# ariloytynoja/pagan2-msa

Measured on AMD Instinct MI355X. Metric: DP cells/sec, 32x100 kb DNA progressive align (hot path in dependency order: fill + traceback per tree level), higher is better.
Workload: dtype f64; 1 GPU; cfg4_32x100kb_dna_anchored; leaves=32, length=100000, data_type=dna, anchors=prefix, offset 15, node_alignments=31, order=guide-tree levels one after the other (a parent needs its children)

## Files before the change

### include/pagan_dp.h

```cpp
#ifndef PAGAN_DP_H
#define PAGAN_DP_H

#include <stdint.h>

#ifdef __cplusplus
extern "C" {
#endif

#define PAGAN_OK              0
#define PAGAN_E_ARG          -1
#define PAGAN_E_GRAPH        -2
#define PAGAN_E_BAND         -3
#define PAGAN_E_MODEL        -4
#define PAGAN_E_NODEVICE     -5
#define PAGAN_E_NOMEM        -6
#define PAGAN_E_INTERNAL     -7
#define PAGAN_DP_REACHED      0
#define PAGAN_DP_UNREACHABLE  1

#define PAGAN_OPT_NO_TERMINAL_EDGES        1u
#define PAGAN_OPT_NO_REDUCED_TERMINAL_PEN  2u

enum { PAGAN_X_MAT = 0, PAGAN_Y_MAT = 1, PAGAN_M_MAT = 2 };
enum { PAGAN_MATCHED = 2, PAGAN_XGAPPED = 3, PAGAN_YGAPPED = 4,
// ... 80 lines not shown

typedef struct pagan_batch pagan_batch;

int  pagan_batch_create(int32_t n, const pagan_job *jobs, const pagan_opts *opts,
                        pagan_batch **out);
int  pagan_batch_run(pagan_batch *b);
int  pagan_batch_sync(pagan_batch *b);
int  pagan_batch_fetch(pagan_batch *b, pagan_result *out );
int  pagan_batch_last_ms(pagan_batch *b, double ms[2]);
int  pagan_batch_last_ms_detail(pagan_batch *b, double ms[6]);
int64_t pagan_batch_cells(const pagan_batch *b);
void pagan_batch_destroy(pagan_batch *b);
int  pagan_batch_debug_trace(pagan_batch *b, int32_t k, void *dst, int64_t bytes);
int  pagan_dp_debug_plan(const pagan_graph *left, const pagan_graph *right, const pagan_band *band,
                         uint8_t *cls, int32_t n_cls, int32_t *sched, int32_t sched_cap, int32_t *sched_len,
                         int32_t *lead_req );
int  pagan_dp_debug_far(const pagan_graph *left, const pagan_graph *right, const pagan_band *band,
                        uint8_t *hfL, uint8_t *hfR, uint8_t *hbit, uint8_t *cls);
int  pagan_dp_debug_strips(const pagan_graph *left, const pagan_graph *right, const pagan_band *band, int32_t max_sites,
                           int32_t *strips , int32_t cap, int64_t *desc_off ,
                           int64_t *desc , int64_t desc_cap);
int  pagan_dp_debug_tiles(const pagan_graph *left, const pagan_graph *right, const pagan_band *band,
                          int32_t *tiles , int32_t cap, int32_t *tile_side);
int  pagan_dp_debug_tiles_staircase(const int32_t *tiles, int32_t n);
int  pagan_dp_debug_compact(const pagan_graph *left, const pagan_graph *right, const pagan_band *band, int32_t *keep_left,
                            int32_t *keep_right, int32_t *slot_left, int32_t *slot_right, int32_t *upper, int32_t *lower,
                            int32_t *n_out);
int  pagan_dp_debug_route(const pagan_graph *left, const pagan_graph *right, const pagan_model *model, const pagan_band *band,
                          int32_t *n_out);
int  pagan_batch_debug_scores(pagan_batch *b, int32_t k, double *dst, int64_t count);
int  pagan_batch_debug_backptrs(pagan_batch *b, int32_t k, uint32_t *dst, int64_t count);
int  pagan_batch_debug_poison(pagan_batch *b);
int  pagan_batch_debug_followed(pagan_batch *b, int32_t k, int32_t *counts);
int  pagan_batch_debug_poke_bp(pagan_batch *b, int32_t k, int32_t i, int32_t j, int32_t vit, uint32_t word);
int  pagan_batch_debug_reruns(pagan_batch *b);

void    pagan_dp_release_cache(void);
int64_t pagan_dp_cached_device_bytes(int32_t device);

typedef struct pagan_model_prob {
    int32_t      n_states;
    const float *score;
    float        gap_open;
    float        gap_ext;
    float        non_gap;
} pagan_model_prob;

typedef struct pagan_fb pagan_fb;

int  pagan_fb_run(const pagan_graph *left, const pagan_graph *right, const pagan_model_prob *model,
                  const pagan_band *band, const pagan_opts *opts, pagan_fb **out);
int  pagan_fb_run_batch(int32_t n, const pagan_graph *const *left, const pagan_graph *const *right,
                        const pagan_model_prob *const *model, const pagan_band *const *band, const pagan_opts *opts,
                        pagan_fb **out);
int  pagan_fb_totals(const pagan_fb *fb, double *log_fwd, double *log_bwd, int64_t *cells);
int  pagan_fb_kernel_ms(const pagan_fb *fb, double ms[2]);
int  pagan_fb_groups(const pagan_fb *fb);
int  pagan_fb_schedule(const pagan_fb *fb);
int  pagan_fb_debug_route(const pagan_graph *left, const pagan_graph *right, const pagan_band *band, int32_t info[8]);
int  pagan_fb_dump(pagan_fb *fb, int32_t which, double *dst);
int  pagan_fb_posterior_cells(pagan_fb *fb, int32_t n, const int32_t *cells, double *post);
int  pagan_fb_sample_path(pagan_fb *fb, const double *u, int32_t n_u, pagan_result *out,
                          int32_t *visited, int32_t *n_visited);
void pagan_fb_destroy(pagan_fb *fb);

const char *pagan_dp_version(void);
// ... 6 lines not shown
```

### pagan2-msa_amd/__init__.py

```python
import ctypes as C
import os

from . import abi
from .abi import Band, Graph, Model, ModelProb, Result

_HERE = os.path.dirname(os.path.abspath(__file__))
LIB_PATH = os.environ.get("PAGAN_DP_LIB") or os.path.join(_HERE, "libpagan_dp.so")
_lib = None


class PaganError(RuntimeError):
    def __init__(self, code, what):
        super().__init__("%s failed with code %d" % (what, code))
        self.code = code


def lib():
    global _lib
    if _lib is None:
        if not os.path.exists(LIB_PATH):
            raise RuntimeError("libpagan_dp.so is missing: run `python -c 'import __graft_entry__ as g; g.build()'`")
        _lib = abi.declare(C.CDLL(LIB_PATH))
    return _lib

# ... 268 lines not shown
        ms = (C.c_double * 2)()
        _check(self._L.pagan_batch_last_ms(self._h, ms), "pagan_batch_last_ms")
        return ms[0], ms[1]

    def fetch(self):
        res = (abi.CResult * self.n)()
        rc = self._L.pagan_batch_fetch(self._h, res)
        try:
            _check(rc, "pagan_batch_fetch")
            return [Result(r) for r in res]
        finally:
            for r in res:
                self._L.pagan_result_free(C.byref(r))

    def debug_scores(self, k):
        import numpy as np
        out = np.empty((self.cells_of(k), 3), np.float64)
        _check(self._L.pagan_batch_debug_scores(self._h, k, out.ctypes.data_as(C.POINTER(C.c_double)), out.size),
               "pagan_batch_debug_scores")
        return out

    def debug_backptrs(self, k):
        import numpy as np
        out = np.empty((self.cells_of(k), 3), np.uint32)
        _check(self._L.pagan_batch_debug_backptrs(self._h, k, out.ctypes.data_as(C.POINTER(C.c_uint32)), out.size),
               "pagan_batch_debug_backptrs")
        return out

    def debug_followed(self, k):
        c = (C.c_int32 * 2)()
        _check(self._L.pagan_batch_debug_followed(self._h, k, c), "pagan_batch_debug_followed")
        return int(c[0]), int(c[1])

    def debug_poke_bp(self, k, i, j, vit, word):
        _check(self._L.pagan_batch_debug_poke_bp(self._h, k, i, j, vit, word), "pagan_batch_debug_poke_bp")

    def debug_reruns(self):
        return int(self._L.pagan_batch_debug_reruns(self._h))

    def debug_trace(self, k, n_cells):
        import numpy as np
        out = np.empty((n_cells, 3), np.int32)
        _check(self._L.pagan_batch_debug_trace(self._h, k, out.ctypes.data_as(C.c_void_p), out.nbytes), "pagan_batch_debug_trace")
        return out

    def cells_of(self, k):
        left, right, _, band = self.jobs[k]
        return self._L.pagan_dp_count_cells(left.n_sites, right.n_sites, C.byref(band.c) if band is not None else None)

    def close(self):
        if self._h:
            self._L.pagan_batch_destroy(self._h)
            self._h = C.c_void_p()

    def __del__(self):
        try:
            self.close()
        except Exception:
            pass
```

### pagan2-msa_amd/abi.py

```python
import ctypes as C

import numpy as np

PAGAN_OK = 0
PAGAN_E_ARG, PAGAN_E_GRAPH, PAGAN_E_BAND, PAGAN_E_MODEL = -1, -2, -3, -4
PAGAN_E_NODEVICE, PAGAN_E_NOMEM, PAGAN_E_INTERNAL = -5, -6, -7
PAGAN_DP_REACHED, PAGAN_DP_UNREACHABLE = 0, 1
OPT_NO_TERMINAL_EDGES = 1
OPT_NO_REDUCED_TERMINAL_PEN = 2
X_MAT, Y_MAT, M_MAT = 0, 1, 2
MATCHED, XGAPPED, YGAPPED, XSKIPPED, YSKIPPED = 2, 3, 4, 5, 6

_i32p = C.POINTER(C.c_int32)
_f32p = C.POINTER(C.c_float)


class CGraph(C.Structure):
    _fields_ = [("n_sites", C.c_int32), ("n_edges", C.c_int32), ("state", _i32p), ("bwd_off", _i32p),
                ("bwd_src", _i32p), ("bwd_logw", _f32p), ("bwd_eid", _i32p)]


class CModel(C.Structure):
    _fields_ = [("n_states", C.c_int32), ("log_score", _f32p), ("log_gap_open", C.c_float),
                ("log_gap_ext", C.c_float), ("log_gap_end_ext", C.c_float), ("log_non_gap", C.c_float)]
# ... 145 lines not shown
    lib.pagan_batch_sync.restype = C.c_int
    lib.pagan_batch_fetch.argtypes = [C.c_void_p, rp]
    lib.pagan_batch_fetch.restype = C.c_int
    lib.pagan_batch_last_ms.argtypes = [C.c_void_p, C.POINTER(C.c_double)]
    lib.pagan_batch_last_ms.restype = C.c_int
    lib.pagan_batch_last_ms_detail.argtypes = [C.c_void_p, C.POINTER(C.c_double)]
    lib.pagan_batch_last_ms_detail.restype = C.c_int
    lib.pagan_batch_cells.argtypes = [C.c_void_p]
    lib.pagan_batch_cells.restype = C.c_int64
    lib.pagan_batch_destroy.argtypes = [C.c_void_p]
    lib.pagan_batch_destroy.restype = None
    lib.pagan_batch_debug_trace.argtypes = [C.c_void_p, C.c_int32, C.c_void_p, C.c_int64]
    lib.pagan_batch_debug_trace.restype = C.c_int
    lib.pagan_dp_debug_plan.argtypes = [gp, gp, bp, C.POINTER(C.c_uint8), C.c_int32, _i32p, C.c_int32, _i32p, _i32p]
    lib.pagan_dp_debug_plan.restype = C.c_int
    lib.pagan_dp_debug_far.argtypes = [gp, gp, bp] + [C.POINTER(C.c_uint8)] * 4
    lib.pagan_dp_debug_far.restype = C.c_int
    lib.pagan_dp_debug_strips.argtypes = [gp, gp, bp, C.c_int32, _i32p, C.c_int32, C.POINTER(C.c_int64), C.POINTER(C.c_int64), C.c_int64]
    lib.pagan_dp_debug_strips.restype = C.c_int
    lib.pagan_dp_debug_tiles.argtypes = [gp, gp, bp, _i32p, C.c_int32, _i32p]
    lib.pagan_dp_debug_tiles.restype = C.c_int
    lib.pagan_dp_debug_compact.argtypes = [gp, gp, bp, _i32p, _i32p, _i32p, _i32p, _i32p, _i32p, _i32p]
    lib.pagan_dp_debug_compact.restype = C.c_int
    lib.pagan_dp_debug_tiles_staircase.argtypes = [_i32p, C.c_int32]
    lib.pagan_dp_debug_tiles_staircase.restype = C.c_int
    lib.pagan_dp_debug_route.argtypes = [gp, gp, C.POINTER(CModel), bp, _i32p]
    lib.pagan_dp_debug_route.restype = C.c_int
    lib.pagan_batch_debug_scores.argtypes = [C.c_void_p, C.c_int32, C.POINTER(C.c_double), C.c_int64]
    lib.pagan_batch_debug_scores.restype = C.c_int
    lib.pagan_batch_debug_backptrs.argtypes = [C.c_void_p, C.c_int32, C.POINTER(C.c_uint32), C.c_int64]
    lib.pagan_batch_debug_backptrs.restype = C.c_int
    lib.pagan_batch_debug_followed.argtypes = [C.c_void_p, C.c_int32, C.POINTER(C.c_int32)]
    lib.pagan_batch_debug_followed.restype = C.c_int
    lib.pagan_batch_debug_poke_bp.argtypes = [C.c_void_p, C.c_int32, C.c_int32, C.c_int32, C.c_int32, C.c_uint32]
    lib.pagan_batch_debug_poke_bp.restype = C.c_int
    lib.pagan_batch_debug_reruns.argtypes = [C.c_void_p]
    lib.pagan_batch_debug_reruns.restype = C.c_int
    lib.pagan_batch_debug_poison.argtypes = [C.c_void_p]
    lib.pagan_batch_debug_poison.restype = C.c_int
    lib.pagan_dp_release_cache.argtypes = []
    lib.pagan_dp_release_cache.restype = None
    lib.pagan_dp_cached_device_bytes.argtypes = [C.c_int32]
    lib.pagan_dp_cached_device_bytes.restype = C.c_int64
    mpp, f64p = C.POINTER(CModelProb), C.POINTER(C.c_double)
    lib.pagan_fb_run.argtypes = [gp, gp, mpp, bp, op, C.POINTER(C.c_void_p)]
    lib.pagan_fb_run.restype = C.c_int
    lib.pagan_fb_run_batch.argtypes = [C.c_int32, C.POINTER(gp), C.POINTER(gp), C.POINTER(mpp), C.POINTER(bp), op, C.POINTER(C.c_void_p)]
    lib.pagan_fb_run_batch.restype = C.c_int
    lib.pagan_fb_totals.argtypes = [C.c_void_p, f64p, f64p, C.POINTER(C.c_int64)]
    lib.pagan_fb_totals.restype = C.c_int
    lib.pagan_fb_kernel_ms.argtypes = [C.c_void_p, C.POINTER(C.c_double)]
    lib.pagan_fb_kernel_ms.restype = C.c_int
    lib.pagan_fb_groups.argtypes = [C.c_void_p]
    lib.pagan_fb_groups.restype = C.c_int
    lib.pagan_fb_schedule.argtypes = [C.c_void_p]
    lib.pagan_fb_schedule.restype = C.c_int
    lib.pagan_fb_debug_route.argtypes = [gp, gp, bp, _i32p]
    lib.pagan_fb_debug_route.restype = C.c_int
    lib.pagan_fb_dump.argtypes = [C.c_void_p, C.c_int32, f64p]
    lib.pagan_fb_dump.restype = C.c_int
    lib.pagan_fb_posterior_cells.argtypes = [C.c_void_p, C.c_int32, _i32p, f64p]
    lib.pagan_fb_posterior_cells.restype = C.c_int
    lib.pagan_fb_sample_path.argtypes = [C.c_void_p, f64p, C.c_int32, rp, _i32p, _i32p]
    lib.pagan_fb_sample_path.restype = C.c_int
    lib.pagan_fb_destroy.argtypes = [C.c_void_p]
    lib.pagan_fb_destroy.restype = None
    lib.pagan_dp_version.argtypes = []
    lib.pagan_dp_version.restype = C.c_char_p
    return lib


EXPORTED = ["pagan_dp_align", "pagan_dp_align_batch", "pagan_result_free", "pagan_dp_predict_bytes",
            "pagan_dp_count_cells", "pagan_dp_device_count", "pagan_dp_select_device", "pagan_batch_create",
            "pagan_batch_run", "pagan_batch_sync", "pagan_batch_fetch", "pagan_batch_last_ms",
            "pagan_batch_cells", "pagan_batch_last_ms_detail", "pagan_batch_destroy", "pagan_batch_debug_trace", "pagan_dp_debug_plan", "pagan_dp_debug_far", "pagan_dp_debug_strips", "pagan_dp_debug_tiles", "pagan_dp_debug_compact", "pagan_dp_debug_tiles_staircase", "pagan_dp_release_cache", "pagan_dp_cached_device_bytes", "pagan_dp_debug_route", "pagan_batch_debug_scores", "pagan_batch_debug_backptrs", "pagan_batch_debug_poison", "pagan_batch_debug_followed", "pagan_batch_debug_poke_bp", "pagan_batch_debug_reruns",
            "pagan_fb_run", "pagan_fb_run_batch", "pagan_fb_totals", "pagan_fb_kernel_ms", "pagan_fb_groups", "pagan_fb_schedule", "pagan_fb_debug_route", "pagan_fb_dump", "pagan_fb_posterior_cells", "pagan_fb_sample_path",
            "pagan_fb_destroy", "pagan_dp_version"]
```

### pagan2-msa_amd/csrc/dp_abi.hip

```cpp
#include <hip/hip_runtime.h>

#include <algorithm>
#include <atomic>
#include <thread>
#include <chrono>
#include <cmath>
#include <cstdint>
#include <cstdio>
#include <cstdlib>
#include <cstring>
#include <condition_variable>
#include <mutex>
#include <new>
#include <type_traits>
#include <vector>
#include <unordered_map>

#include "host_anchors.h"
#include "host_graph.h"
#include "../../include/pagan_dp.h"
#include "dp_device.h"
#include "dp_band.h"

template <int BLOCK> __global__ void pg_fill_wavefront(const PgDevJob *jobs, const int *which, unsigned flags);
// ... 1007 lines not shown
        if (!p) return;
        std::lock_guard<std::mutex> g(m);
        idle.emplace_back(p, cap);
    }
};
StagePool stage_pool;
struct Stage {
    char *p = nullptr;
    size_t cap = 0;
    explicit Stage(size_t n) { p = stage_pool.take(n, &cap); }
    ~Stage() { stage_pool.give(p, cap); }
    Stage(const Stage &) = delete;
    Stage &operator=(const Stage &) = delete;
    char *data() { return p; }
};

template <class T> void put(Stage &stage, const void *devptr_as_off, const T *src, size_t count) {
    if (count) std::memcpy(stage.data() + reinterpret_cast<size_t>(devptr_as_off), src, sizeof(T) * count);
}

static int bp_diags_per_block(int max_nd, int other_dims) {
    int dpb = PG_BP_DIAGS;
    while (dpb > 4 && (long long)((max_nd + dpb - 1) / dpb) * other_dims < 4096) dpb /= 2;
    return dpb;
}

int launch_fill(pagan_batch *b) {
    unsigned chk_banded = PG_FLAG_SCORE_CHECK, chk_wide = b->n_striped > 0 ? PG_FLAG_SCORE_CHECK : 0u;
    if (const char *e = std::getenv("PAGAN_DP_SCORE_CHECK")) {
        if (std::strcmp(e, "0") == 0) { chk_banded = 0; chk_wide = 0; }
        else if (std::strcmp(e, "all") == 0) chk_wide = PG_FLAG_SCORE_CHECK;
    }
    const unsigned spread = b->strips_spread ? PG_FLAG_STRIPS_SPREAD : 0u;
    hipStream_t tile_stream = nullptr;
    static std::atomic<int> n_cu_dev[64];
    bool ev3_recorded = false;
    if (b->n_striped > 0 && b->strips_alone) {
        HIP_TRY(hipMemsetAsync(b->arena.dev + b->sfollow_begin, 0, b->sfollow_bytes, b->stream));
        if (b->strip_grid > 0)
            hipLaunchKernelGGL((pg_fill_pipe<true, true>), dim3(b->strip_grid), dim3(pg_pipe_block()), 0, b->stream,
                               b->d_jobs, b->d_swhich, ((b->flags & 0x400u) ? b->flags : (b->flags & ~0x800u)) | spread, b->strip_grid);
        if (b->strip_grid_big > 0)
            hipLaunchKernelGGL((pg_fill_pipe<false, true>), dim3(b->strip_grid_big), dim3(pg_pipe_block()), 0, b->stream,
                               b->d_jobs, b->d_swhich + b->strip_grid, ((b->flags & 0x400u) ? b->flags : (b->flags & ~0x800u)) | spread, b->strip_grid_big);
    }
    if (b->n_striped > 0 && b->tile_off.size() <= 1) {
        hipStream_t st = b->stream;
        if (b->stream2) {
            HIP_TRY(hipEventRecord(b->ev_fork, b->stream));
            HIP_TRY(hipStreamWaitEvent(b->stream2, b->ev_fork, 0));
            st = b->stream2;
        }
        tile_stream = st;
    }
    if (b->tile_off.size() > 1) {
        static std::atomic<bool> tiles_set_dev[64];
        std::atomic<bool> &tiles_set = tiles_set_dev[b->device & 63];
        if (!tiles_set.load()) {
            HIP_TRY(hipFuncSetAttribute(reinterpret_cast<const void *>(pg_fill_tiles),
                                        hipFuncAttributeMaxDynamicSharedMemorySize, (int)pg_tiles_lds_bytes()));
            HIP_TRY(hipFuncSetAttribute(reinterpret_cast<const void *>(pg_fill_tiles_flow),
                                        hipFuncAttributeMaxDynamicSharedMemorySize, (int)pg_tiles_lds_bytes()));
            int n_cu = 0;
            HIP_TRY(hipDeviceGetAttribute(&n_cu, hipDeviceAttributeMultiprocessorCount, b->device));
            n_cu_dev[b->device & 63].store(n_cu > 0 ? n_cu : 256);
            tiles_set.store(true);
        }
        hipStream_t st = b->stream;
        if (b->stream2) {
            HIP_TRY(hipEventRecord(b->ev_fork, b->stream));
            HIP_TRY(hipStreamWaitEvent(b->stream2, b->ev_fork, 0));
            st = b->stream2;
        }
        tile_stream = st;
    }
    if (b->n_ring > 0) {
        static std::atomic<bool> lds_set_dev[64];
        std::atomic<bool> &lds_set = lds_set_dev[b->device & 63];
        if (!lds_set.load()) {
            HIP_TRY(hipFuncSetAttribute(reinterpret_cast<const void *>(pg_fill_ring<true>),
                                        hipFuncAttributeMaxDynamicSharedMemorySize, (int)pg_ring_lds_bytes()));
            HIP_TRY(hipFuncSetAttribute(reinterpret_cast<const void *>(pg_fill_ring<false>),
                                        hipFuncAttributeMaxDynamicSharedMemorySize, (int)pg_ring_lds_bytes()));
            lds_set.store(true);
        }
        const int n_small = b->n_ring_small, n_big = b->n_ring - b->n_ring_small;
        HIP_TRY(hipEventRecord(b->evk[0], b->stream)); b->evk_set[0] = true;
        if (b->use_pipe) {
            bool follow = b->bp_pass == 1 && b->follow_bytes > 0 && !b->no_follow;
            if (const char *f = std::getenv("PAGAN_DP_FOLLOW")) follow = follow && std::strcmp(f, "0") != 0;
            if (b->follow_bytes > 0) HIP_TRY(hipMemsetAsync(b->arena.dev + b->follow_begin, 0, b->follow_bytes, b->stream));
            auto followers = [&](int n_fill) { return follow && n_fill <= 32 ? std::min(96, 48 * ((n_fill + 7) / 8)) : 0; };
            if (n_small > 0)
                hipLaunchKernelGGL((pg_fill_pipe<true, false>), dim3(n_small + followers(n_small)), dim3(pg_pipe_block()), 0 , b->stream,
                                   b->d_jobs, b->d_which, b->flags | chk_banded, n_small);
            if (n_big > 0)
                hipLaunchKernelGGL((pg_fill_pipe<false, false>), dim3(n_big + followers(n_big)), dim3(pg_pipe_block()), 0, b->stream,
                                   b->d_jobs, b->d_which + n_small, b->flags | chk_banded, n_big);
            HIP_TRY(hipEventRecord(b->evk[1], b->stream)); b->evk_set[1] = true;
            if (b->bp_pass) {
                int max_nd = 1, max_w = 1;
                for (int k = 0; k < b->n; ++k) if (b->jobs[k].ring_ok) { max_nd = std::max(max_nd, b->dj[k].nd); max_w = std::max(max_w, b->jobs[k].dx.max_width); }
                const int zc = (max_w + PG_BP_CELLS - 1) / PG_BP_CELLS, dpb = bp_diags_per_block(max_nd, b->n_ring * zc);
                hipLaunchKernelGGL(pg_backptr, dim3((max_nd + dpb - 1) / dpb, b->n_ring, zc), dim3(256), 0, b->stream,
                                   b->d_jobs, b->d_which, (b->flags & 0xffu) | (b->bp_pass == 2 ? 0x100u : chk_banded), dpb);
                HIP_TRY(hipEventRecord(b->evk[2], b->stream)); b->evk_set[2] = true;
            }
        } else {
            b->evk_set[1] = false;
            if (n_small > 0)
                hipLaunchKernelGGL(pg_fill_ring<true>, dim3(n_small), dim3(576), pg_ring_lds_bytes(), b->stream,
                                   b->d_jobs, b->d_which, b->flags);
            if (n_big > 0)
                hipLaunchKernelGGL(pg_fill_ring<false>, dim3(n_big), dim3(576), pg_ring_lds_bytes(), b->stream,
                                   b->d_jobs, b->d_which + n_small, b->flags);
        }
    }
    if (b->n_wide > 0) {
        dim3 grid(b->n_wide);
        const int *which = b->d_which + b->n_ring;
        switch (b->block) {
        case 64: hipLaunchKernelGGL(pg_fill_wavefront<64>, grid, dim3(64), 0, b->stream, b->d_jobs, which, b->flags); break;
        case 256: hipLaunchKernelGGL(pg_fill_wavefront<256>, grid, dim3(256), 0, b->stream, b->d_jobs, which, b->flags); break;
        default: hipLaunchKernelGGL(pg_fill_wavefront<1024>, grid, dim3(1024), 0, b->stream, b->d_jobs, which, b->flags); break;
        }
        HIP_TRY(hipEventRecord(b->evk[5], b->stream)); b->evk_set[5] = true;
    }
    if (b->n_striped > 0 && !b->strips_alone) {
        HIP_TRY(hipEventRecord(b->evk[3], tile_stream)); b->evk_set[3] = true; ev3_recorded = true;
        HIP_TRY(hipMemsetAsync(b->arena.dev + b->sfollow_begin, 0, b->sfollow_bytes, tile_stream));
        if (b->strip_grid > 0)
// ... 934 lines not shown
    });
    int first_err = PAGAN_OK;
    for (int k = 0; k < b->n; ++k)
        if (rcs[k] != PAGAN_OK && first_err == PAGAN_OK) first_err = rcs[k];
    return first_err;
}

int pagan_batch_debug_poison(pagan_batch *b) {
    if (!b) return PAGAN_E_ARG;
    HIP_TRY(hipMemsetAsync(b->arena.dev + b->out_begin, 0xFF, b->arena.size - b->out_begin, b->stream));
    return PAGAN_OK;
}

int pagan_batch_debug_poke_bp(pagan_batch *b, int32_t k, int32_t i, int32_t j, int32_t vit, uint32_t word) {
    if (!b || k < 0 || k >= b->n) return PAGAN_E_ARG;
    b->poke[0] = k; b->poke[1] = i; b->poke[2] = j; b->poke[3] = vit; b->poke[4] = (int)word;
    return PAGAN_OK;
}
int pagan_batch_debug_reruns(pagan_batch *b) { return b ? b->reruns : PAGAN_E_ARG; }

int pagan_batch_debug_followed(pagan_batch *b, int32_t k, int32_t *counts) {
    if (!b || k < 0 || k >= b->n || !counts) return PAGAN_E_ARG;
    counts[0] = counts[1] = 0;
    if (!b->dj[k].bp_done) return PAGAN_OK;
    HIP_TRY(hipStreamSynchronize(b->stream));
    const size_t n = ((size_t)b->dj[k].nd + PG_FOLLOW_CHUNK - 1) / PG_FOLLOW_CHUNK;
    std::vector<unsigned char> flags(n);
    HIP_TRY(hipMemcpy(flags.data(), b->dj[k].bp_done, n, hipMemcpyDeviceToHost));
    counts[1] = (int32_t)n;
    for (unsigned char f : flags) counts[0] += f != 0;
    return PAGAN_OK;
}

int pagan_batch_debug_scores(pagan_batch *b, int32_t k, double *dst, int64_t count) {
    if (!b || k < 0 || k >= b->n || !dst || count > 3 * b->jobs[k].dx.cells) return PAGAN_E_ARG;
    HIP_TRY(hipStreamSynchronize(b->stream));
    HIP_TRY(hipMemcpy(dst, b->dj[k].sc, sizeof(double) * (size_t)count, hipMemcpyDeviceToHost));
    return PAGAN_OK;
}

int pagan_batch_debug_backptrs(pagan_batch *b, int32_t k, uint32_t *dst, int64_t count) {
    if (!b || k < 0 || k >= b->n || !dst || count > 3 * b->jobs[k].dx.cells) return PAGAN_E_ARG;
    HIP_TRY(hipStreamSynchronize(b->stream));
    HIP_TRY(hipMemcpy(dst, b->dj[k].bp, sizeof(uint32_t) * (size_t)count, hipMemcpyDeviceToHost));
    return PAGAN_OK;
}

int pagan_batch_debug_trace(pagan_batch *b, int32_t k, void *dst, int64_t bytes) {
    if (!b || k < 0 || k >= b->n || !dst) return PAGAN_E_ARG;
    HIP_TRY(hipStreamSynchronize(b->stream));
    HIP_TRY(hipMemcpy(dst, b->arena.dev + b->trace_off[k], (size_t)bytes, hipMemcpyDeviceToHost));
    return PAGAN_OK;
}

void pagan_batch_destroy(pagan_batch *b) {
    if (!b) return;
    if (b->stream) {
        (void)hipStreamSynchronize(b->stream);
        if (b->pooled_stream2) (void)hipStreamSynchronize(b->pooled_stream2);
        GpuObjs o;
        o.stream = b->stream; o.stream2 = b->pooled_stream2; o.ev_fork = b->pooled_fork; o.ev_join = b->pooled_join;
        for (int k = 0; k < 3; ++k) o.ev[k] = b->ev[k];
        for (int k = 0; k < 7; ++k) o.evk[k] = b->evk[k];
        gpu_pool.give(b->device, o);
    }
    if (b->arena.dev) arena_pool.give(b->device, b->arena.dev, b->arena.cap);
// ... 85 lines not shown
```

### pagan2-msa_amd/csrc/dp_device.h

```cpp
#pragma once
#include <stdint.h>

#define PG_BP_NONE 3u
#define PG_BP_ADJL 4u
#define PG_BP_ADJR 8u
#define PG_MAX_SLOT 16383
#define PG_SEG 256
#define PG_BP_DIAGS 64
#define PG_BP_CELLS 1024
#define PG_STATUS_PATH_CHECK 3
#define PG_FLAG_SCORE_CHECK 0x200u
#define PG_FLAG_STRIPS_SPREAD 0x10000u
#define PG_FILL_SCORE_MISMATCH 0x7c
#define PG_FILL_OTHER_XCD 0x20000000
#define PG_FOLLOW_CHUNK 16

#define PG_PIPE_WIDTH 242
#define PG_PIPE_REACH 14
#define PG_PIPE_RING 14
#define PG_HIST_SLOTS 3
#define PG_HIST_MAX_SPAN 44
#define PG_PIPE_ASSIST 3
#define PG_PIPE_STAGE 3
#define PG_PIPE_WAKE 6
#define PG_PIPE_WINDOW 432
#define PG_PIPE_WINDOW_A 352
#define PG_PIPE_EDGE_CAP 1024
#define PG_PIPE_SITE_EDGES 126

#define PG_TILE 64
#define PG_TILE_EDGES 512

struct PgDevJob {
    int Lx, Ly;
    int nd;
    int S;
    float go, ge, gE, ng;
    const int *stL, *offL, *srcL; const float *lwL;
    const int *stR, *offR, *srcR; const float *lwR;
    const float *table;
    const int *imin, *imax;
    const long long *doff;
    const int *dsc;
    const int *psc;
    const int *sched;
// ... 28 lines not shown
```

### pagan2-msa_amd/csrc/dp_pipe.hip

```cpp
#include "dp_kcommon.h"
#include <type_traits>

#define PNW 4
#define PNT (64 * PNW)
#define PNTW PG_PIPE_WIDTH
#define PRK PG_PIPE_RING
#define PAGE PG_PIPE_REACH
#define PRW 512
#define PEC PG_PIPE_EDGE_CAP
#define PDR 128
#define PDR_REACH 60
#define PLOOK 64
#define PLAND 8
#define PNA PG_PIPE_ASSIST
#define PST PG_PIPE_STAGE
#define PBLOCK (PNT + 64 * PNA + 64)
static_assert(PNTW == PNT - PAGE && PRK >= PAGE && PG_PIPE_WINDOW + 80 <= PRW, "kernel geometry out of step with dp_device.h");
static_assert(PNA == 3 && PST == 3 && PAGE >= PLAND + 4, "assist wave a stages the diagonals d % 3 == a into slot a, at most two diagonals ahead; far cells have landed");
#define PFAR_POOL ((PNT * 4) / 24)
#define PS_ONLY 0x80000000u
#define PS_FIRST 0x40000000u
#define PS_BP 0x3fffffffu
#ifndef PG_SPIN_LIMIT_LOG2
#define PG_SPIN_LIMIT_LOG2 25
// ... 2166 lines not shown
    asm volatile("s_waitcnt vmcnt(0)" ::: "memory");
    flag_store(&PM.wflag[w7], d0 - 1);
    flag_store(&PM.warrived[w7], d0);
    for (int w = 0; w < PW7; ++w) POLLX(&PM.warrived[w], d0, 7);
    p_up = d0 - 1 > p_up ? d0 - 1 : p_up;
    p_dn = d0 - 1 > p_dn ? d0 - 1 : p_dn;
    int run_end = d0 + 1;
    for (;;) {
        const int t = run_end + lane;
        const int c4 = ((PG_GLOBAL const int *)psc)[8 * (t < nd ? t : nd) + 4] & 15;
        const unsigned long long stop = __builtin_amdgcn_ballot_w64(t >= nd || c4 != 4);
        if (stop != 0) { run_end += __builtin_ctzll(stop); break; }
        run_end += 64;
    }
    asm volatile("s_waitcnt vmcnt(0)" ::: "memory");
    pg_i4 cur = {dA.x, dA.y, dA.z, dA.w};
    int wr;
    { int m_ = (tid - cur.x) % PW7L; m_ += m_ < 0 ? PW7L : 0; wr = cur.x + m_; }
    if (diags_ld < d0) diags_ld = POLLX(&PM.loaded[2], d0, 5);
    double Px, Py, Pm, Cx, Cy, Cm, Ux, Uy, Um;
    {
        const FarAsk fP = far_ask(psc, d0, 1, wr), fC = far_ask(psc, d0, 2, wr - 1), fU = far_ask(psc, d0, 1, wr - 1), none = {false, 0};
        pg_d2 a = {NIw, NIw}, b = {NIw, NIw}, c = {NIw, NIw}, e = {NIw, NIw};
        double ma = NIw, mb = NIw, mc = NIw, me = NIw;
        far_fetch4(sc_out, fP, fC, fU, none, a, ma, b, mb, c, mc, e, me);
        Px = a.x; Py = a.y; Pm = ma; Cx = b.x; Cy = b.y; Cm = mb; Ux = c.x; Uy = c.y; Um = mc;
    }
    const bool geo_b = (dA.s4 & 16) != 0;
    const int wpos_n = geo_b ? PWPOS_B : PWPOS_A, wk = geo_b ? PWK_B : PWK_A, wage = wk - 2, wrow_bytes = wpos_n * 24;
    int wbase = cur.x - 32;
    auto wpos = [&](int r_) { int q_ = r_ - wbase; q_ -= q_ >= wpos_n ? wpos_n : 0; q_ -= q_ >= wpos_n ? wpos_n : 0; return q_; };
    int n_hist1 = 0, n_hist2 = 0;
    int lo_prev = cur.x;
    for (;;) {
        const int lo = cur.x, hi = cur.y;
        if (lo - 2 * wage - 4 - wbase >= wpos_n) wbase += wpos_n;
#ifdef PG_PIPE_STATS
        const long long st_step0 = __builtin_readcyclecounter();
#endif
        {
            const int nr_ = hi + 1 < Lx ? hi + 1 : Lx, nc_ = d - lo + 1 < Ly ? d - lo + 1 : Ly;
            if (rows_ld < nr_) rows_ld = POLLX(&PM.loaded[0], nr_, 1);
            if (cols_ld < nc_) cols_ld = POLLX(&PM.loaded[1], nc_, 2);
            if (diags_ld < d) diags_ld = POLLX(&PM.loaded[2], d, 5);
        }
        const int r = wr < lo ? wr + PW7L : wr, j = d - r;
        int kind = 0;
        pg_i4 gl = {0, 0, 0, 0}, gr = {0, 0, 0, 0};
        bool l2 = false, r2 = false, l3 = false, r3 = false;
        int kL = 1, kR = 1, kL3 = 1, kR3 = 1;
        double lwA = 0, lwS = 0, lwT = 0, rwA = 0, rwS = 0, rwT = 0;
        double tM = 0, tX = 0;
        if (r <= hi) {
            gl = PM.recL[r & (PRW - 1)]; gr = PM.recR[j & (PRW - 1)];
            const int nl = (gl.x >> PR_NE_SHIFT) & 127, nr = (gr.x >> PR_NE_SHIFT) & 127;
            auto shape = [&](auto left_tag, const pg_i4 &rec, int site, int n, bool &two, bool &three, int &k1, int &k3, double &wA, double &w1, double &w3) -> bool {
                constexpr bool LEFT = decltype(left_tag)::value;
                const int e0 = rec.y & 0xffff, e1 = (int)((unsigned)rec.y >> 16);
                const double f0 = (double)__int_as_float(rec.z), f1 = (double)__int_as_float(rec.w);
                two = false; three = false; k1 = 1; k3 = 1; wA = f0; w1 = 0.0; w3 = 0.0;
                if (n == 1) return e0 == 1;
                if (n == 2) {
                    two = true;
                    if (e0 == 1) { wA = f0; k1 = e1; w1 = f1; } else { wA = f1; k1 = e0; w1 = f0; }
                    return (e0 == 1) != (e1 == 1);
                }
                if (n == 3) {
                    int e2; double f2;
                    edge_at<LEFT>(rec, 2, site, e2, f2);
                    two = true; three = true;
                    if (e0 == 1) { wA = f0; k1 = e1; w1 = f1; k3 = e2; w3 = f2; }
                    else if (e1 == 1) { wA = f1; k1 = e0; w1 = f0; k3 = e2; w3 = f2; }
                    else { wA = f2; k1 = e0; w1 = f0; k3 = e1; w3 = f1; }
                    return ((e0 == 1) + (e1 == 1) + (e2 == 1)) == 1;
                }
                return false;
            };
            bool l2_, l3_, r2_, r3_;
// ... 164 lines not shown
            double *o = (double *)((char *)&PM.sc[0][0][0] + wsb + wpos(wr) * 24);
            o[PG_X] = bx; o[PG_Y] = by; o[PG_M] = bm;
        }
        if (__any(kind != 0 && ((gl.x | gr.x) & PR_SRC))) { if (kind != 0) hist_append(gl, gr, r, j, bx, by, bm); }
        if (wpos_n > PW7L && wr < lo + wpos_n - PW7L) {
            double *o = (double *)((char *)&PM.sc[0][0][0] + wsb + wpos(wr + PW7L) * 24);
            o[PG_X] = NIw; o[PG_Y] = NIw; o[PG_M] = NIw;
        }
        {
            const int tot = n_hist1 + n_hist2;
            if (tot >= 4) asm volatile("s_waitcnt vmcnt(4)" ::: "memory");
            else if (tot >= 2) asm volatile("s_waitcnt vmcnt(2)" ::: "memory");
            else asm volatile("s_waitcnt vmcnt(0)" ::: "memory");
            n_hist2 = n_hist1; n_hist1 = n_now;
        }
        flag_store(&PM.wflag[w7], d);
        if (w7 < PNW) flag_store(&PM.progress[w7], d);
        if (active) {
            const unsigned off24 = __umul24((unsigned)(wr - lo), 24u);
            pg_d2 xy; xy.x = bx; xy.y = by;
            *(PG_GLOBAL pg_d2 *)(srow + off24) = xy;
            *(PG_GLOBAL double *)(srow + off24 + 16u) = bm;
        }
        Px = bx; Py = by; Pm = bm;
        Cx = Ux; Cy = Uy; Cm = Um;
#ifdef PG_PIPE_STATS
        if (w7 < PNW) {
            const long long st_t5 = __builtin_readcyclecounter();
            st_cls_t[4] += st_t5 - st_step0; ++st_cls_n[4];
            st_w[0] += st_t1 - st_step0; st_w[1] += st_t2 - st_t1; st_w[2] += st_t3 - st_t2; st_w[3] += st_t5 - st_t3;
        }
#endif
        ++d;
        lo_prev = lo;
        if (d >= run_end || flag_load(&PM.abort_flag) != 0) break;
        cur.x = __builtin_amdgcn_readfirstlane(nxt.x); cur.y = __builtin_amdgcn_readfirstlane(nxt.y);
        cur.z = __builtin_amdgcn_readfirstlane(nxt.z); cur.w = __builtin_amdgcn_readfirstlane(nxt.w);
    }
    asm volatile("s_waitcnt vmcnt(0)" ::: "memory");
    flag_store(&PM.warrived[w7], d);
    for (int w = 0; w < PW7; ++w) POLLX(&PM.warrived[w], d, 7);
    dA = psc[d];
    row = dA.x + ((tid - dA.x) & (PNT - 1));
    ok_until = d - 1;
    C_.dA = dA;
    WCTX_OUT(C_);
}

__device__ __noinline__ void widest_run7(WaveCtx &C_) {
    WCTX_IN(C_);
    WCTX_STATS(C_);
    const PgDevJob *__restrict__ job = (const PgDevJob *)uniform_u64((unsigned long long)C_.job);
    const unsigned flags_ = __builtin_amdgcn_readfirstlane(C_.flags);
    const bool no_terminal_edges = flags_ & 1u, reduced_terminal = !(flags_ & 2u);
    pg_i8 dA = uniform_i8(C_.dA);
    const int d0 = d;
    const int lane = tid & 63, w7 = wave;
    asm volatile("s_waitcnt vmcnt(0)" ::: "memory");
    flag_store(&PM.wflag[w7], d0 - 1);
    flag_store(&PM.warrived[w7], d0);
    for (int w = 0; w < PW7; ++w) POLLX(&PM.warrived[w], d0, 7);
    p_up = d0 - 1 > p_up ? d0 - 1 : p_up;
    p_dn = d0 - 1 > p_dn ? d0 - 1 : p_dn;
    int run_end = d0 + 1;
    for (;;) {
        const int t = run_end + lane;
        const int c5 = ((PG_GLOBAL const int *)psc)[8 * (t < nd ? t : nd) + 4] & 15;
        const unsigned long long stop = __builtin_amdgcn_ballot_w64(t >= nd || c5 != 5);
        if (stop != 0) { run_end += __builtin_ctzll(stop); break; }
        run_end += 64;
    }
    asm volatile("s_waitcnt vmcnt(0)" ::: "memory");
// ... 701 lines not shown
```

Before: 591.8 million cells/s.

## Add fast-path step for easy inner cells in wide pipelined fill

```diff
diff --git a/include/pagan_dp.h b/include/pagan_dp.h
--- a/include/pagan_dp.h
+++ b/include/pagan_dp.h
@@ -136,6 +136,7 @@
 int  pagan_batch_debug_backptrs(pagan_batch *b, int32_t k, uint32_t *dst, int64_t count);
 int  pagan_batch_debug_poison(pagan_batch *b);
 int  pagan_batch_debug_followed(pagan_batch *b, int32_t k, int32_t *counts);
+int  pagan_batch_debug_wide_fast(pagan_batch *b, int32_t k, int32_t *steps);
 int  pagan_batch_debug_poke_bp(pagan_batch *b, int32_t k, int32_t i, int32_t j, int32_t vit, uint32_t word);
 int  pagan_batch_debug_reruns(pagan_batch *b);
 
diff --git a/pagan2-msa_amd/__init__.py b/pagan2-msa_amd/__init__.py
--- a/pagan2-msa_amd/__init__.py
+++ b/pagan2-msa_amd/__init__.py
@@ -324,6 +324,11 @@
         _check(self._L.pagan_batch_debug_followed(self._h, k, c), "pagan_batch_debug_followed")
         return int(c[0]), int(c[1])
 
+    def debug_wide_fast(self, k):
+        c = C.c_int32(0)
+        _check(self._L.pagan_batch_debug_wide_fast(self._h, k, C.byref(c)), "pagan_batch_debug_wide_fast")
+        return int(c.value)
+
     def debug_poke_bp(self, k, i, j, vit, word):
         _check(self._L.pagan_batch_debug_poke_bp(self._h, k, i, j, vit, word), "pagan_batch_debug_poke_bp")
 
diff --git a/pagan2-msa_amd/abi.py b/pagan2-msa_amd/abi.py
--- a/pagan2-msa_amd/abi.py
+++ b/pagan2-msa_amd/abi.py
@@ -201,6 +201,9 @@
     lib.pagan_batch_debug_backptrs.restype = C.c_int
     lib.pagan_batch_debug_followed.argtypes = [C.c_void_p, C.c_int32, C.POINTER(C.c_int32)]
     lib.pagan_batch_debug_followed.restype = C.c_int
+    if hasattr(lib, "pagan_batch_debug_wide_fast"):
+        lib.pagan_batch_debug_wide_fast.argtypes = [C.c_void_p, C.c_int32, C.POINTER(C.c_int32)]
+        lib.pagan_batch_debug_wide_fast.restype = C.c_int
     lib.pagan_batch_debug_poke_bp.argtypes = [C.c_void_p, C.c_int32, C.c_int32, C.c_int32, C.c_int32, C.c_uint32]
     lib.pagan_batch_debug_poke_bp.restype = C.c_int
     lib.pagan_batch_debug_reruns.argtypes = [C.c_void_p]
@@ -242,6 +245,6 @@
 EXPORTED = ["pagan_dp_align", "pagan_dp_align_batch", "pagan_result_free", "pagan_dp_predict_bytes",
             "pagan_dp_count_cells", "pagan_dp_device_count", "pagan_dp_select_device", "pagan_batch_create",
             "pagan_batch_run", "pagan_batch_sync", "pagan_batch_fetch", "pagan_batch_last_ms",
-            "pagan_batch_cells", "pagan_batch_last_ms_detail", "pagan_batch_destroy", "pagan_batch_debug_trace", "pagan_dp_debug_plan", "pagan_dp_debug_far", "pagan_dp_debug_strips", "pagan_dp_debug_tiles", "pagan_dp_debug_compact", "pagan_dp_debug_tiles_staircase", "pagan_dp_release_cache", "pagan_dp_cached_device_bytes", "pagan_dp_debug_route", "pagan_batch_debug_scores", "pagan_batch_debug_backptrs", "pagan_batch_debug_poison", "pagan_batch_debug_followed", "pagan_batch_debug_poke_bp", "pagan_batch_debug_reruns",
+            "pagan_batch_cells", "pagan_batch_last_ms_detail", "pagan_batch_destroy", "pagan_batch_debug_trace", "pagan_dp_debug_plan", "pagan_dp_debug_far", "pagan_dp_debug_strips", "pagan_dp_debug_tiles", "pagan_dp_debug_compact", "pagan_dp_debug_tiles_staircase", "pagan_dp_release_cache", "pagan_dp_cached_device_bytes", "pagan_dp_debug_route", "pagan_batch_debug_scores", "pagan_batch_debug_backptrs", "pagan_batch_debug_poison", "pagan_batch_debug_followed", "pagan_batch_debug_wide_fast", "pagan_batch_debug_poke_bp", "pagan_batch_debug_reruns",
             "pagan_fb_run", "pagan_fb_run_batch", "pagan_fb_totals", "pagan_fb_kernel_ms", "pagan_fb_groups", "pagan_fb_schedule", "pagan_fb_debug_route", "pagan_fb_dump", "pagan_fb_posterior_cells", "pagan_fb_sample_path",
             "pagan_fb_destroy", "pagan_dp_version"]
diff --git a/pagan2-msa_amd/csrc/dp_abi.hip b/pagan2-msa_amd/csrc/dp_abi.hip
--- a/pagan2-msa_amd/csrc/dp_abi.hip
+++ b/pagan2-msa_amd/csrc/dp_abi.hip
@@ -1063,6 +1063,8 @@
         else if (std::strcmp(e, "all") == 0) chk_wide = PG_FLAG_SCORE_CHECK;
     }
     const unsigned spread = b->strips_spread ? PG_FLAG_STRIPS_SPREAD : 0u;
+    unsigned wide_fast = 0u;
+    if (const char *e = std::getenv("PAGAN_DP_WIDE_FAST")) { if (std::strcmp(e, "0") == 0) wide_fast = PG_FLAG_WIDE_FAST_OFF; }
     hipStream_t tile_stream = nullptr;
     static std::atomic<int> n_cu_dev[64];
     bool ev3_recorded = false;
@@ -1124,10 +1126,10 @@
             auto followers = [&](int n_fill) { return follow && n_fill <= 32 ? std::min(96, 48 * ((n_fill + 7) / 8)) : 0; };
             if (n_small > 0)
                 hipLaunchKernelGGL((pg_fill_pipe<true, false>), dim3(n_small + followers(n_small)), dim3(pg_pipe_block()), 0 , b->stream,
-                                   b->d_jobs, b->d_which, b->flags | chk_banded, n_small);
+                                   b->d_jobs, b->d_which, b->flags | chk_banded | wide_fast, n_small);
             if (n_big > 0)
                 hipLaunchKernelGGL((pg_fill_pipe<false, false>), dim3(n_big + followers(n_big)), dim3(pg_pipe_block()), 0, b->stream,
-                                   b->d_jobs, b->d_which + n_small, b->flags | chk_banded, n_big);
+                                   b->d_jobs, b->d_which + n_small, b->flags | chk_banded | wide_fast, n_big);
             HIP_TRY(hipEventRecord(b->evk[1], b->stream)); b->evk_set[1] = true;
             if (b->bp_pass) {
                 int max_nd = 1, max_w = 1;
@@ -2128,6 +2130,15 @@
     return PAGAN_OK;
 }
 
+int pagan_batch_debug_wide_fast(pagan_batch *b, int32_t k, int32_t *steps) {
+    if (!b || k < 0 || k >= b->n || !steps) return PAGAN_E_ARG;
+    *steps = 0;
+    if (!b->dj[k].follow) return PAGAN_OK;
+    HIP_TRY(hipStreamSynchronize(b->stream));
+    HIP_TRY(hipMemcpy(steps, b->dj[k].follow + 3, sizeof(int32_t), hipMemcpyDeviceToHost));
+    return PAGAN_OK;
+}
+
 int pagan_batch_debug_scores(pagan_batch *b, int32_t k, double *dst, int64_t count) {
     if (!b || k < 0 || k >= b->n || !dst || count > 3 * b->jobs[k].dx.cells) return PAGAN_E_ARG;
     HIP_TRY(hipStreamSynchronize(b->stream));
diff --git a/pagan2-msa_amd/csrc/dp_device.h b/pagan2-msa_amd/csrc/dp_device.h
--- a/pagan2-msa_amd/csrc/dp_device.h
+++ b/pagan2-msa_amd/csrc/dp_device.h
@@ -11,6 +11,7 @@
 #define PG_STATUS_PATH_CHECK 3
 #define PG_FLAG_SCORE_CHECK 0x200u
 #define PG_FLAG_STRIPS_SPREAD 0x10000u
+#define PG_FLAG_WIDE_FAST_OFF 0x20000u
 #define PG_FILL_SCORE_MISMATCH 0x7c
 #define PG_FILL_OTHER_XCD 0x20000000
 #define PG_FOLLOW_CHUNK 16
diff --git a/pagan2-msa_amd/csrc/dp_pipe.hip b/pagan2-msa_amd/csrc/dp_pipe.hip
--- a/pagan2-msa_amd/csrc/dp_pipe.hip
+++ b/pagan2-msa_amd/csrc/dp_pipe.hip
@@ -2222,6 +2222,10 @@
     auto wpos = [&](int r_) { int q_ = r_ - wbase; q_ -= q_ >= wpos_n ? wpos_n : 0; q_ -= q_ >= wpos_n ? wpos_n : 0; return q_; };
     int n_hist1 = 0, n_hist2 = 0;
     int lo_prev = cur.x;
+    int wslot = d0 % wk;
+    int n_fast = 0;
+    const bool fast_on = !(flags_ & PG_FLAG_WIDE_FAST_OFF);
+    (void)wslot; (void)n_fast; (void)fast_on;
     for (;;) {
         const int lo = cur.x, hi = cur.y;
         if (lo - 2 * wage - 4 - wbase >= wpos_n) wbase += wpos_n;
@@ -2234,6 +2238,144 @@
             if (cols_ld < nc_) cols_ld = POLLX(&PM.loaded[1], nc_, 2);
             if (diags_ld < d) diags_ld = POLLX(&PM.loaded[2], d, 5);
         }
+#if !defined(PG_EXP_WIDE_SKIP) && !defined(PG_NO_WIDE_FAST)
+        if (fast_on && d > d0) {
+            if (diags_ld < d + 2 && d + 1 < nd) diags_ld = POLLX(&PM.loaded[2], d + 2, 5);
+            const int r = wr < lo ? wr + PW7L : wr, j = d - r;
+            const bool act = r <= hi;
+            const pg_i4 gl = PM.recL[r & (PRW - 1)], gr = PM.recR[j & (PRW - 1)];
+            const pg_i4 nxt = PM.dring[(d + 1) & (PDR - 1)];
+            const int *fp = &PM.wflag[0] + (lane < PW7 ? lane : (int)((offsetof(PipeSmem, abort_flag) - offsetof(PipeSmem, wflag)) / sizeof(int)));
+            int fv = flag_peek(fp);
+            const bool l2 = (gl.x & (PR_TWO | PR_THREE)) == PR_TWO, r2 = (gr.x & (PR_TWO | PR_THREE)) == PR_TWO;
+            const int nl = (gl.x >> PR_NE_SHIFT) & 127, nr = (gr.x >> PR_NE_SHIFT) & 127;
+            const int kL = l2 ? (int)((unsigned)gl.y >> 16) : 1, kR = r2 ? (int)((unsigned)gr.y >> 16) : 1;
+            const bool easy = (l2 || (nl == 1 && (gl.y & 0xffff) == 1)) && (r2 || (nr == 1 && (gr.y & 0xffff) == 1));
+            const bool inner = r >= 2 && r <= Lx - 2 && j >= 2 && j <= Ly - 2 && r - kL >= 1 && j - kR >= 1;
+            const int amax = d - d0 < wage ? d - d0 : wage;
+            const int oldest = l2 ? (r2 ? kL + kR : kL + 1) : (r2 ? kR + 1 : 0);
+            if (__builtin_amdgcn_ballot_w64(act && !(easy && inner && oldest <= amax)) != 0) goto compiled_step;
+            {
+                const int want = lane == up7 ? d - 1 : d - 2;
+                int looks = 0;
+                unsigned long long bad;
+                for (;;) {
+                    bad = __builtin_amdgcn_ballot_w64(lane < PW7 ? fv < want : fv != 0);
+                    if (bad == 0 || ++looks > 24) break;
+                    fv = flag_peek(fp);
+                }
+                if (bad != 0) goto compiled_step;
+            }
+#ifdef PG_PIPE_STATS
+            const long long st_t1 = __builtin_readcyclecounter();
+#endif
+            const double lwA = (double)__int_as_float(gl.z), lwS = l2 ? (double)__int_as_float(gl.w) : 0.0;
+            const double rwA = (double)__int_as_float(gr.z), rwS = r2 ? (double)__int_as_float(gr.w) : 0.0;
+            const unsigned long long anyL = __builtin_amdgcn_ballot_w64(act && l2), anyR = __builtin_amdgcn_ballot_w64(act && r2);
+            const int wsb = wslot * wrow_bytes, ring_bytes = wk * wrow_bytes;
+            const char *ring = (const char *)&PM.sc[0][0][0];
+            const int null_off = (int)offsetof(PipeSmem, null_cell) - (int)offsetof(PipeSmem, sc);
+            const int pos = wpos(r);
+            int pos1 = pos - 1; pos1 += pos1 < 0 ? wpos_n : 0;
+            int posL = pos - kL; posL += posL < 0 ? wpos_n : 0;
+            auto cell_off = [&](bool need, int age, int p24) {
+                int rb = wsb - age * wrow_bytes;
+                rb += rb < 0 ? ring_bytes : 0;
+                return need ? rb + p24 : null_off;
+            };
+            const int ti_ = ((gl.x & 0xffff) + __umul24(gr.x & 0xffff, S)) & 255;
+            const double tM = PM.tab2[ti_][0], tX = PM.tab2[ti_][1];
+            const double *cu = (const double *)(ring + cell_off(true, 1, pos1 * 24));
+            const double ux_ = cu[PG_X], uy_ = cu[PG_Y], um_ = cu[PG_M];
+            pg_d2 lx_ = {NIw, NIw}, lm_ = {NIw, NIw}, ry_ = {NIw, NIw}, rm_ = {NIw, NIw}, lr_ = {NIw, NIw};
+            double lxm = NIw, lmm = NIw, rym = NIw, rmm = NIw, lrm = NIw;
+            if (anyL != 0) {
+                const bool nl2 = act && l2;
+                const double *c3 = (const double *)(ring + cell_off(nl2, kL, posL * 24)), *c4 = (const double *)(ring + cell_off(nl2, kL + 1, posL * 24));
+                lx_.x = c3[PG_X]; lx_.y = c3[PG_Y]; lxm = c3[PG_M];
+                lm_.x = c4[PG_X]; lm_.y = c4[PG_Y]; lmm = c4[PG_M];
+                if ((anyL & anyR) != 0) {
+                    const double *c7 = (const double *)(ring + cell_off(nl2 && r2, kL + kR, posL * 24));
+                    lr_.x = c7[PG_X]; lr_.y = c7[PG_Y]; lrm = c7[PG_M];
+                }
+            }
+            if (anyR != 0) {
+                const bool nr2 = act && r2;
+                const double *c5 = (const double *)(ring + cell_off(nr2, kR, pos * 24)), *c6 = (const double *)(ring + cell_off(nr2, kR + 1, pos1 * 24));
+                ry_.x = c5[PG_X]; ry_.y = c5[PG_Y]; rym = c5[PG_M];
+                rm_.x = c6[PG_X]; rm_.y = c6[PG_Y]; rmm = c6[PG_M];
+            }
+            {
+                const double ax = dpp_shr1(Px, ux_), ay = dpp_shr1(Py, uy_), am = dpp_shr1(Pm, um_);
+                const bool top = wr == lo_prev;
+                Ux = top ? NIw : ax; Uy = top ? NIw : ay; Um = top ? NIw : am;
+                if (wr < lo) { wr += PW7L; Px = NIw; Py = NIw; Pm = NIw; Cx = NIw; Cy = NIw; Cm = NIw; Ux = NIw; Uy = NIw; Um = NIw; }
+            }
+            double bx = NIw, by = NIw, bm = NIw;
+            if (act) {
+                auto gapv = [&](double own, double other, double m_) { return __builtin_fmax(own + ge, __builtin_fmax(other, m_ + ng) + go); };
+                auto pairv = [&](double x_, double y_, double m_, double lw, double rw) {
+                    return (__builtin_fmax(m_ + tM, __builtin_fmax(x_, y_) + tX) + lw) + rw;
+                };
+                bx = gapv(Ux, Uy, Um);
+                by = gapv(Py, Px, Pm);
+                bm = pairv(Cx, Cy, Cm, lwA, rwA);
+                if (anyR != 0) {
+                    by = __builtin_fmax(by, gapv(ry_.y, ry_.x, rym));
+                    bm = __builtin_fmax(bm, pairv(rm_.x, rm_.y, rmm, lwA, rwS));
+                }
+                if (anyL != 0) {
+                    bx = __builtin_fmax(bx, gapv(lx_.x, lx_.y, lxm));
+                    bm = __builtin_fmax(bm, pairv(lm_.x, lm_.y, lmm, lwS, rwA));
+                    if ((anyL & anyR) != 0) bm = __builtin_fmax(bm, pairv(lr_.x, lr_.y, lrm, lwS, rwS));
+                }
+            }
+            if (wr < lo + wpos_n) {
+                double *o = (double *)((char *)&PM.sc[0][0][0] + wsb + pos * 24);
+                o[PG_X] = bx; o[PG_Y] = by; o[PG_M] = bm;
+            }
+            if (__any(act && ((gl.x | gr.x) & PR_SRC))) { if (act) hist_append(gl, gr, r, j, bx, by, bm); }
+            if (wpos_n > PW7L && wr < lo + wpos_n - PW7L) {
+                double *o = (double *)((char *)&PM.sc[0][0][0] + wsb + wpos(wr + PW7L) * 24);
+                o[PG_X] = NIw; o[PG_Y] = NIw; o[PG_M] = NIw;
+            }
+            {
+                const int tot = n_hist1 + n_hist2;
+                if (tot >= 4) asm volatile("s_waitcnt vmcnt(4)" ::: "memory");
+                else if (tot >= 2) asm volatile("s_waitcnt vmcnt(2)" ::: "memory");
+                else asm volatile("s_waitcnt vmcnt(0)" ::: "memory");
+                n_hist2 = n_hist1; n_hist1 = __any(act) ? 2 : 0;
+            }
+            flag_store_inorder(&PM.wflag[w7], d);
+            if (w7 < PNW) flag_store_inorder(&PM.progress[w7], d);
+            if (act) {
+                const long long soff = ((long long)cur.w << 32) | (unsigned)cur.z;
+                PG_GLOBAL char *srow = (PG_GLOBAL char *)sc_out + soff;
+                const unsigned off24 = __umul24((unsigned)(wr - lo), 24u);
+                pg_d2 xy; xy.x = bx; xy.y = by;
+                *(PG_GLOBAL pg_d2 *)(srow + off24) = xy;
+                *(PG_GLOBAL double *)(srow + off24 + 16u) = bm;
+            }
+            Px = bx; Py = by; Pm = bm;
+            Cx = Ux; Cy = Uy; Cm = Um;
+#ifdef PG_PIPE_STATS
+            if (w7 < PNW) {
+                const long long st_t5 = __builtin_readcyclecounter();
+                st_cls_t[4] += st_t5 - st_step0; ++st_cls_n[4];
+                st_w[0] += st_t1 - st_step0; st_w[3] += st_t5 - st_t1;
+            }
+#endif
+            ++n_fast;
+            ++d;
+            wslot = wslot + 1 == wk ? 0 : wslot + 1;
+            lo_prev = lo;
+            if (d >= run_end) break;
+            cur.x = __builtin_amdgcn_readfirstlane(nxt.x); cur.y = __builtin_amdgcn_readfirstlane(nxt.y);
+            cur.z = __builtin_amdgcn_readfirstlane(nxt.z); cur.w = __builtin_amdgcn_readfirstlane(nxt.w);
+            continue;
+        }
+compiled_step:
+#endif
         const int r = wr < lo ? wr + PW7L : wr, j = d - r;
         int kind = 0;
         pg_i4 gl = {0, 0, 0, 0}, gr = {0, 0, 0, 0};
@@ -2464,12 +2606,14 @@
         }
 #endif
         ++d;
+        wslot = wslot + 1 == wk ? 0 : wslot + 1;
         lo_prev = lo;
         if (d >= run_end || flag_load(&PM.abort_flag) != 0) break;
         cur.x = __builtin_amdgcn_readfirstlane(nxt.x); cur.y = __builtin_amdgcn_readfirstlane(nxt.y);
         cur.z = __builtin_amdgcn_readfirstlane(nxt.z); cur.w = __builtin_amdgcn_readfirstlane(nxt.w);
     }
     asm volatile("s_waitcnt vmcnt(0)" ::: "memory");
+    if (n_fast > 0 && lane == 0 && job->follow) __hip_atomic_fetch_add((PG_GLOBAL int *)job->follow + 3, n_fast, __ATOMIC_RELAXED, __HIP_MEMORY_SCOPE_AGENT);
     flag_store(&PM.warrived[w7], d);
     for (int w = 0; w < PW7; ++w) POLLX(&PM.warrived[w], d, 7);
     dA = psc[d];
```

After: 585.0 million cells/s. 0.988x the previous value.
